# tum-pbs/PhiFlow

Hardware: NVIDIA H100
Metric: smoke_plume_512^3_steps_per_sec (higher is better)
Workload: dtype f32

## Files before the change

### phiflow_b200/csrc/ring_kernels.cu

```cuda
#include <cooperative_groups.h>
#include <type_traits>
#include "cg_common.cuh"
#include <cstdlib>
#include <cstring>
#include "launch.cuh"

namespace cg = cooperative_groups;

#define RING_CONSUMERS 256
#define RING_THREADS (RING_CONSUMERS + 32)
#define RING_MAX_STAGES 8
#define RING_G 4

struct RingCfg {
    int TY, R, pitch, nx4;
    int stage_floats;
    int ZC, nyt, nzc;
    int units_per_batch, total_units;
    int consumers;
    int groups;
    int shfl_ok;
    int hint;
    int merge;
    int dbg;
// ... 677 lines not shown
    {
        const float4 m = make_float4(c.x + q.x, c.y + q.y, c.z + q.z, c.w + q.w);
        e(off, c, m, nvalid, e0, e1, e2);
    }
};

template <int DIM, bool AXPY, bool GENERIC>
__global__ void __launch_bounds__(RING_THREADS, 2)
k_laplace_ring(DGrid g, DField f, RingCfg cfg, const float* __restrict__ x, float* __restrict__ y, float coeff)
{
    extern __shared__ __align__(128) unsigned char smem[];
    Ring rg;
    ring_init(rg, smem, cfg);
    ThreadGroups tg;
    groups_init(tg, cfg, g, f);
    const float* hsrc[2] = {x, nullptr};
    const float* esrc[2] = {nullptr, nullptr};
    REpiLaplace<AXPY> epi{y, coeff};
    for (int unit = blockIdx.x; unit < cfg.total_units; unit += gridDim.x) {
        const RingUnit u = ring_unit<DIM>(cfg, g, unit);
        ring_process_unit<GENERIC, DIM, 1, 0, false>(rg, cfg, g, f, tg, hsrc, esrc, 0.f, u, epi);
    }
}

struct CgRingArgs {
    CgArgs a;
    RingCfg cfg;
    int ring_smem_offset;
    int comm_merge;
    CommDev cm;
    float* d2;
    CgOperator op;
};

template <int DIM, bool GENERIC, CgOp OP, int NH, int NE, class Epi>
__device__ __forceinline__ void cg_op_unit(Ring& rg, const CgRingArgs& A, ThreadGroups& tg, const float* const* hsrc,
                                           const float* const* esrc, float beta, const RingUnit& u, Epi& epi)
{
    if constexpr (OP == CgOp::Helmholtz) {
        REpiHelm<Epi> he{epi, A.op.amount};
        ring_process_unit<GENERIC, DIM, NH, NE, true, OP>(rg, A.cfg, A.a.g, A.a.pf, tg, hsrc, esrc, beta, u, he);
    } else if constexpr (OP == CgOp::HelmholtzVarying) {
        REpiVarHelm<Epi> he{epi};
        ring_process_unit<GENERIC, DIM, NH, NE, true, OP>(rg, A.cfg, A.a.g, A.a.pf, tg, hsrc, esrc, beta, u, he, A.op.kbcast ? 0 : u.b, &A.op);
    } else ring_process_unit<GENERIC, DIM, NH, NE, true, OP>(rg, A.cfg, A.a.g, A.a.pf, tg, hsrc, esrc, beta, u, epi);
}

__device__ __forceinline__ unsigned long long ld_acquire_sys(const unsigned long long* p)
{
    unsigned long long v;
    asm volatile("ld.acquire.sys.global.u64 %0, [%1];" : "=l"(v) : "l"(p) : "memory");
    return v;
}
__device__ __forceinline__ void st_release_sys(unsigned long long* p, unsigned long long v)
{
    asm volatile("st.release.sys.global.u64 [%0], %1;" ::"l"(p), "l"(v) : "memory");
}

__device__ __forceinline__ bool comm_allreduce(const CommDev& cm, const CgShared& sh, int batch, unsigned long long seq)
{
    const int par = (int)(seq & 1ull);
    const size_t stride = 2 * (size_t)CG_MAX_BATCH;
    if (blockIdx.x == 0) {
        for (int q = 0; q < cm.n; ++q) {
            double* dst = cm.mbox[q] + ((size_t)par * PHI_MAX_RANKS + cm.rank) * stride;
            for (int b = threadIdx.x; b < batch; b += blockDim.x) { dst[b] = sh.sum0[b]; dst[CG_MAX_BATCH + b] = sh.sum1[b]; }
        }
        __threadfence_system();
        __syncthreads();
        if ((int)threadIdx.x < cm.n) st_release_sys(cm.flag[threadIdx.x] + par * PHI_MAX_RANKS + cm.rank, seq);
    }
    bool ok = true;
    if ((int)threadIdx.x < cm.n) {
        const unsigned long long* f = cm.flag[cm.rank] + par * PHI_MAX_RANKS + threadIdx.x;
        const long long t0 = clock64();
        while (ld_acquire_sys(f) < seq) {
            if (clock64() - t0 > 40000000000ll) { ok = false; break; }
        }
    }
    ok = __syncthreads_and(ok);
    const double* src = cm.mbox[cm.rank] + (size_t)par * PHI_MAX_RANKS * stride;
    for (int b = threadIdx.x; b < batch; b += blockDim.x) {
        double s0 = 0, s1 = 0;
        for (int q = 0; q < cm.n; ++q) {
            s0 += *(volatile const double*)(src + q * stride + b);
            s1 += *(volatile const double*)(src + q * stride + CG_MAX_BATCH + b);
        }
        sh.sum0[b] = s0; sh.sum1[b] = s1;
    }
    __syncthreads();
    return ok;
}

__device__ __forceinline__ bool comm_barrier_allreduce(const CommDev& cm, const CgShared& sh, const double* partials, int region, int batch,
                                                       int units_per_batch, const unsigned char* active, unsigned long long seq)
{
    const int par = (int)(seq & 1ull);
    const size_t stride = 2 * (size_t)CG_MAX_BATCH;
    __threadfence_system();
    __syncthreads();
    if (threadIdx.x == 0) {
        const unsigned prev = atomicAdd(cm.arrive, 1u);
        sh.any_cont[1] = ((prev + 1u) % gridDim.x == 0u) ? 1 : 0;
    }
    __syncthreads();
    if (sh.any_cont[1]) {
        __threadfence();
        reduce_partials(sh, partials, region, batch, units_per_batch, active);
        for (int q = 0; q < cm.n; ++q) {
            double* dst = cm.mbox[q] + ((size_t)par * PHI_MAX_RANKS + cm.rank) * stride;
            for (int b = threadIdx.x; b < batch; b += blockDim.x) { dst[b] = sh.sum0[b]; dst[CG_MAX_BATCH + b] = sh.sum1[b]; }
        }
        __threadfence_system();
        __syncthreads();
        if ((int)threadIdx.x < cm.n) st_release_sys(cm.flag[threadIdx.x] + par * PHI_MAX_RANKS + cm.rank, seq);
    }
    bool ok = true;
    if ((int)threadIdx.x < cm.n) {
        const unsigned long long* f = cm.flag[cm.rank] + par * PHI_MAX_RANKS + threadIdx.x;
        const long long t0 = clock64();
        while (ld_acquire_sys(f) < seq) {
            if (clock64() - t0 > 40000000000ll) { ok = false; break; }
        }
    }
    ok = __syncthreads_and(ok);
    const double* src = cm.mbox[cm.rank] + (size_t)par * PHI_MAX_RANKS * stride;
    for (int b = threadIdx.x; b < batch; b += blockDim.x) {
        double s0 = 0, s1 = 0;
        for (int q = 0; q < cm.n; ++q) {
            s0 += *(volatile const double*)(src + q * stride + b);
            s1 += *(volatile const double*)(src + q * stride + CG_MAX_BATCH + b);
        }
        sh.sum0[b] = s0; sh.sum1[b] = s1;
    }
    __syncthreads();
    return ok;
}

template <int DIM, class F>
__device__ __forceinline__ void ring_unit_cells(const RingCfg& cfg, const DGrid& g, const DField& pf, const ThreadGroups& tg,
                                                const RingUnit& u, F&& fn)
{
    if ((int)threadIdx.x >= cfg.consumers) return;
    long long plane_off = (long long)u.b * pf.sb + (long long)u.y0 * pf.sy + (DIM == 3 ? (long long)u.z0 * pf.sz : 0);
    for (int z = u.z0; z < u.z1; ++z, plane_off += pf.sz)
#pragma unroll
        for (int k = 0; k < RING_G; ++k) {
            if (tg.j[k] < 0 || u.y0 + tg.j[k] >= g.n[1]) continue;
            const int x0 = tg.eoff[k] - tg.j[k] * cfg.pitch;
            fn(plane_off + tg.goff[k], min(4, g.n[0] - x0));
        }
}

#define RING_GF 3
#define FUSED_TILE_BUFS 3

struct FusedGroups {
    int t[RING_GF];
    int tl[RING_GF], tr[RING_GF];
    int goff[RING_GF];
    unsigned valid, inner, needl, needr;
};

__device__ __forceinline__ void fused_groups_init(FusedGroups& fg, const RingCfg& cfg, const DGrid& g, const DField& pf)
{
    const int lane = threadIdx.x & 31, nx = g.n[0], pitch = cfg.pitch;
    fg.valid = fg.inner = fg.needl = fg.needr = 0;
#pragma unroll
    for (int k = 0; k < RING_GF; ++k) {
        const int ge = threadIdx.x + k * cfg.consumers;
        const int jj = ge / cfg.nx4, x0 = (ge - jj * cfg.nx4) * 4;
        const int row = jj * pitch;
        if (jj < cfg.TY + 2) fg.valid |= 1u << k;
        if (jj >= 1 && jj <= cfg.TY) fg.inner |= 1u << k;
        fg.t[k] = row + x0;
        fg.goff[k] = (jj - 1) * (int)pf.sy + x0;
        fg.tl[k] = row + x0 - 1; fg.tr[k] = row + x0 + 4;
        if (lane == 0) fg.needl |= 1u << k;
        if (lane == 31) fg.needr |= 1u << k;
        if (x0 == 0) { fg.needl |= 1u << k; fg.tl[k] = pf.klo[0] == PHI_BC_PERIODIC ? row + nx - 1 : row; }
        if (x0 + 4 >= nx) { fg.needr |= 1u << k; fg.tr[k] = pf.khi[0] == PHI_BC_PERIODIC ? row : row + nx - 1; }
        if (!(fg.needl & (1u << k))) fg.tl[k] = 0;
        if (!(fg.needr & (1u << k))) fg.tr[k] = 0;
    }
}

struct ProdUnitF {
    long long yoff[4];
    const float* base[4];
    uint32_t dsto[4];
    uint32_t nbytes[4];
    unsigned m[3];
    int tot[3];
};

__device__ __forceinline__ void prod_fused_setup(ProdUnitF& pu, const RingCfg& cfg, const DGrid& g, const DField& pf,
                                                 const float* d, const float* dprev, const float* x, int b, int y0)
{
    const int lane = threadIdx.x & 31, TY = cfg.TY;
    const uint32_t row_bytes = (uint32_t)cfg.pitch * 4u;
    const bool mergeable = cfg.merge && pf.sy == cfg.pitch;
    const int rows[3] = {TY + 4, TY + 2, TY};
    const int ylo[3] = {y0 - 2, y0 - 1, y0};
    const float* src[3] = {d, dprev, x};
    int cnt[3] = {0, 0, 0};
    pu.m[0] = pu.m[1] = pu.m[2] = 0;
#pragma unroll
    for (int it = 0; it < 4; ++it) {
        const int line = lane + 32 * it;
        pu.yoff[it] = 0; pu.base[it] = nullptr; pu.dsto[it] = 0; pu.nbytes[it] = row_bytes;
        int key = -1, yv = 0, first = 0;
#pragma unroll
        for (int arr = 0; arr < 3; ++arr) {
            if (key < 0 && line >= first && line < first + rows[arr] && src[arr]) {
                int yy = ylo[arr] + (line - first); float cv;
                phi_resolve(yy, pf, 1, cv);
                pu.yoff[it] = (long long)b * pf.sb + (long long)yy * pf.sy;
                pu.base[it] = src[arr];
                pu.dsto[it] = 4u * (uint32_t)(line * cfg.pitch);
                key = arr; yv = yy;
            }
            first += rows[arr];
        }
        cnt[0] += key == 0; cnt[1] += key == 1; cnt[2] += key == 2;
        const int pkey = __shfl_up_sync(0xffffffffu, key, 1), pyv = __shfl_up_sync(0xffffffffu, yv, 1);
        const bool cont = mergeable && key >= 0 && lane > 0 && pkey == key && pyv + 1 == yv;
        const unsigned cm = __ballot_sync(0xffffffffu, cont);
        if (key >= 0 && !cont) {
            const unsigned follow = lane == 31 ? 0u : (cm >> (lane + 1));
            pu.nbytes[it] = (uint32_t)__ffs(~follow) * row_bytes;
            if (key == 0) pu.m[0] |= 1u << it; else if (key == 1) pu.m[1] |= 1u << it; else pu.m[2] |= 1u << it;
        }
    }
#pragma unroll
    for (int c = 0; c < 3; ++c) {
#pragma unroll
        for (int o = 16; o > 0; o >>= 1) cnt[c] += __shfl_xor_sync(0xffffffffu, cnt[c], o);
        pu.tot[c] = cnt[c];
    }
}

__device__ __forceinline__ void ring_produce_fused(Ring& rg, const RingCfg& cfg, const DField& pf, const ProdUnitF& pu, int z, bool pplane, bool eplane)
{
    const int lane = threadIdx.x & 31;
    const int slot = rg.pos.slot;
    const uint32_t full = rg.full0 + 8 * slot;
    const uint32_t sbase = rg.stage0_s + 4u * (uint32_t)(slot * cfg.stage_floats);
    float cv;
    phi_resolve(z, pf, 2, cv);
    const long long zoff = (long long)z * pf.sz;
    const unsigned mask = pu.m[0] | (pplane ? pu.m[1] : 0u) | (eplane ? pu.m[2] : 0u);
    const int cnt = pu.tot[0] + (pplane ? pu.tot[1] : 0) + (eplane ? pu.tot[2] : 0);
    if (lane == 0) {
        mbar_wait(rg.empty0 + 8 * slot, rg.pos.par ^ 1u);
        mbar_expect_tx(full, (uint32_t)cnt * (uint32_t)cfg.pitch * 4u);
    }
    __syncwarp();
#pragma unroll
    for (int it = 0; it < 4; ++it)
        if (mask & (1u << it)) bulk_g2s(sbase + pu.dsto[it], pu.base[it] + pu.yoff[it] + zoff, pu.nbytes[it], full);
    rg.pos.next(cfg.R);
}

__device__ __forceinline__ float4 lds4(const float* s, int off) { return *reinterpret_cast<const float4*>(s + off); }
__device__ __forceinline__ float dot4(const float4& a, const float4& b) { return a.x * b.x + a.y * b.y + a.z * b.z + a.w * b.w; }

__device__ __forceinline__ float4 stencil7(const float4& c, float xl, float xr, const float4& ym, const float4& yp, const float4& zm, const float4& zp,
                                           float ix2, float iy2, float iz2, float cc)
{
    float4 q;
    q.x = fmaf(ix2, xl + c.y, fmaf(iy2, ym.x + yp.x, -cc * c.x));
    q.y = fmaf(ix2, c.x + c.z, fmaf(iy2, ym.y + yp.y, -cc * c.y));
    q.z = fmaf(ix2, c.y + c.w, fmaf(iy2, ym.z + yp.z, -cc * c.z));
    q.w = fmaf(ix2, c.z + xr, fmaf(iy2, ym.w + yp.w, -cc * c.w));
    q.x = fmaf(iz2, zm.x + zp.x, q.x);
    q.y = fmaf(iz2, zm.y + zp.y, q.y);
    q.z = fmaf(iz2, zm.z + zp.z, q.z);
    q.w = fmaf(iz2, zm.w + zp.w, q.w);
    return q;
}

struct FusedPass {
    const float* d; const float* dprev;
    float* dn; float* x;
    float alpha, aprev, beta, bprev;
};

__device__ __forceinline__ void ring_fused_unit(Ring& rg, const RingCfg& cfg, const DGrid& g, const DField& pf, const FusedGroups& fg,
                                                const FusedPass& P, float* tile, const RingUnit& u, float (&acc)[4])
{
    const int nz = u.z1 - u.z0;
    if ((int)threadIdx.x >= cfg.consumers) {
        ProdUnitF pu;
        prod_fused_setup(pu, cfg, g, pf, P.d, P.dprev, P.x, u.b, u.y0);
        for (int p = 0; p < nz + 4; ++p)
            ring_produce_fused(rg, cfg, pf, pu, u.z0 - 2 + p, p >= 1 && p <= nz + 2, P.x && p >= 2 && p <= nz + 1);
        return;
    }
    const int pitch = cfg.pitch, TY = cfg.TY;
    const int pb = (TY + 4) * pitch, xb = (2 * TY + 6) * pitch - pitch;
    const int tsz = (TY + 2) * pitch;
    const float ix2 = g.inv_dx2[0], iy2 = g.inv_dx2[1], iz2 = g.inv_dx2[2];
    const float cc = 2.f * (ix2 + iy2 + iz2);
    const float alpha = P.alpha, aprev = P.aprev, beta = P.beta, bprev = P.bprev;
    const bool has_prev = P.dprev != nullptr;
    long long plane_off = (long long)u.b * pf.sb + (long long)u.y0 * pf.sy + (long long)u.z0 * pf.sz - pf.sz;

    float4 dm[RING_GF], dc[RING_GF];
    float4 n2[RING_GF], n1[RING_GF];
    float4 r1[RING_GF];
    SlotIt cur = rg.pos, nxt = cur; nxt.next(cfg.R);
    ring_wait_full(rg, cur); ring_wait_full(rg, nxt);
    {
        const float* s0 = ring_ptr(rg, cfg, cur);
        const float* s1 = ring_ptr(rg, cfg, nxt);
#pragma unroll
        for (int k = 0; k < RING_GF; ++k) {
            dm[k] = f4_splat(0.f); dc[k] = f4_splat(0.f);
            if (fg.valid & (1u << k)) { dm[k] = lds4(s0, pitch + fg.t[k]); dc[k] = lds4(s1, pitch + fg.t[k]); }
            n2[k] = n1[k] = r1[k] = f4_splat(0.f);
        }
    }
    ring_release(rg, cur);
    cur = nxt; nxt.next(cfg.R);
    for (int i = 0; i < nz + 2; ++i) {
        const bool own = i >= 1 && i <= nz;
        ring_wait_full(rg, nxt);
        const float* sc = ring_ptr(rg, cfg, cur);
        const float* sn = ring_ptr(rg, cfg, nxt);
        float* tw = tile + (i % FUSED_TILE_BUFS) * tsz;
        float4 n0[RING_GF], r0[RING_GF];
#pragma unroll
        for (int k = 0; k < RING_GF; ++k) {
            n0[k] = r0[k] = f4_splat(0.f);
            if (!(fg.valid & (1u << k))) continue;
            const int o = pitch + fg.t[k];
            const float4 c = dc[k];
            const float4 ym = lds4(sc, o - pitch), yp = lds4(sc, o + pitch), zp = lds4(sn, o);
            float xl = __shfl_up_sync(0xffffffffu, c.w, 1), xr = __shfl_down_sync(0xffffffffu, c.x, 1);
            const float el = sc[pitch + fg.tl[k]], er = sc[pitch + fg.tr[k]];
            xl = (fg.needl & (1u << k)) ? el : xl;
            xr = (fg.needr & (1u << k)) ? er : xr;
            const float4 q = stencil7(c, xl, xr, ym, yp, dm[k], zp, ix2, iy2, iz2, cc);
            float4 rv = c, dp = f4_splat(0.f);
            if (has_prev) {
                dp = lds4(sc, pb + fg.t[k]);
                rv = make_float4(fmaf(-bprev, dp.x, c.x), fmaf(-bprev, dp.y, c.y), fmaf(-bprev, dp.z, c.z), fmaf(-bprev, dp.w, c.w));
            }
            rv.x = fmaf(-alpha, q.x, rv.x); rv.y = fmaf(-alpha, q.y, rv.y); rv.z = fmaf(-alpha, q.z, rv.z); rv.w = fmaf(-alpha, q.w, rv.w);
            const float4 dv = make_float4(fmaf(beta, c.x, rv.x), fmaf(beta, c.y, rv.y), fmaf(beta, c.z, rv.z), fmaf(beta, c.w, rv.w));
            *reinterpret_cast<float4*>(tw + fg.t[k]) = dv;
            if (own && (fg.inner & (1u << k))) {
                const long long off = plane_off + fg.goff[k];
                *reinterpret_cast<float4*>(P.dn + off) = dv;
                acc[1] += dot4(rv, rv);
                if (P.x) {
                    float4 xv = lds4(sc, xb + fg.t[k]);
                    xv.x += aprev * dp.x; xv.y += aprev * dp.y; xv.z += aprev * dp.z; xv.w += aprev * dp.w;
                    xv.x += alpha * c.x; xv.y += alpha * c.y; xv.z += alpha * c.z; xv.w += alpha * c.w;
                    *reinterpret_cast<float4*>(P.x + off) = xv;
                }
            }
            n0[k] = dv; r0[k] = rv;
            dm[k] = c; dc[k] = zp;
        }
        ring_release(rg, cur);
        asm volatile("bar.sync 1, %0;" ::"r"(cfg.consumers) : "memory");
        if (i >= 2) {
            const float* tp = tile + ((i - 1) % FUSED_TILE_BUFS) * tsz;
#pragma unroll
            for (int k = 0; k < RING_GF; ++k) {
                if (!(fg.inner & (1u << k))) continue;
                const float4 c = n1[k];
                const float4 ym = lds4(tp, fg.t[k] - pitch), yp = lds4(tp, fg.t[k] + pitch);
                float xl = __shfl_up_sync(0xffffffffu, c.w, 1), xr = __shfl_down_sync(0xffffffffu, c.x, 1);
                const float el = tp[fg.tl[k]], er = tp[fg.tr[k]];
                xl = (fg.needl & (1u << k)) ? el : xl;
                xr = (fg.needr & (1u << k)) ? er : xr;
                const float4 q = stencil7(c, xl, xr, ym, yp, n2[k], n0[k], ix2, iy2, iz2, cc);
                acc[0] += dot4(c, q);
                acc[2] += dot4(r1[k], q);
                acc[3] += dot4(q, q);
            }
        }
#pragma unroll
        for (int k = 0; k < RING_GF; ++k) { n2[k] = n1[k]; n1[k] = n0[k]; r1[k] = r0[k]; }
        cur = nxt; nxt.next(cfg.R);
        plane_off += pf.sz;
    }
    ring_release(rg, cur);
    rg.pos = nxt;
    asm volatile("bar.sync 1, %0;" ::"r"(cfg.consumers) : "memory");
}

struct REpiFusedStart {
    float* d; float acc0, acc1;
    __device__ __forceinline__ void set_plane(int, int) {}
    __device__ __forceinline__ void set_acc(const float4&) {}
    __device__ __forceinline__ void operator()(long long off, const float4& c, const float4& q, int, const float4&, const float4&, const float4&)
    {
        *reinterpret_cast<float4*>(d + off) = c;
        acc0 += dot4(c, q);
        acc1 += dot4(q, q);
    }
};

template <int DIM, bool GENERIC, bool DIST, bool ADAPT, CgOp OP = CgOp::Poisson, bool FUSED = false>
__global__ void __launch_bounds__(RING_THREADS, 1)
k_cg_ring(CgRingArgs A)
{
    constexpr bool MASK = OP == CgOp::Masked;
    static_assert((OP != CgOp::Helmholtz && OP != CgOp::HelmholtzVarying) || (!DIST && !ADAPT && !FUSED),
                  "the Helmholtz operators run on the single-GPU two-sweep CG only");
    static_assert(!MASK || !ADAPT || (!DIST && !FUSED), "CG-adaptive with obstacles runs on the single-GPU two-sweep CG only");
    static_assert(!cg_op_xslot(OP) || GENERIC, "the face-minimum stencil runs on the generic consumer");
    extern __shared__ __align__(128) unsigned char smem_raw[];
    const CgArgs& a = A.a;
    const RingCfg& cfg = A.cfg;
    CgShared sh = cg_carve(smem_raw, a.g.batch);
    Ring rg;
    ring_init(rg, smem_raw + A.ring_smem_offset, cfg);
    cg::grid_group grid = cg::this_grid();
    const DGrid& g = a.g;
    const int batch = g.batch;
    const double cells = (double)g.n[0] * g.n[1] * g.n[2] * (A.cm.n > 1 ? A.cm.n : 1);
    const float coffs = a.prm.matrix_offset;
    constexpr bool adaptive = ADAPT;
    int region = 0;
    ThreadGroups tg;
    groups_init(tg, cfg, g, a.pf);

    auto sweep = [&](const unsigned char* active, auto&& body) {
        int cur_b = cfg.split ? 0 : -1; float acc0 = 0.f, acc1 = 0.f;
        RingUnit u;
        for (int k = 0; ring_next_unit<DIM>(cfg, g, k, u); ++k) {
            if (active && !active[u.b]) continue;
            if (u.b != cur_b) {
                if (cur_b >= 0) flush_partials(sh, a.partials, region, batch, cur_b, acc0, acc1);
                cur_b = u.b; acc0 = 0.f; acc1 = 0.f;
            }
            body(u, acc0, acc1);
        }
        if (cur_b >= 0) flush_partials(sh, a.partials, region, batch, cur_b, acc0, acc1);
    };
    const CommDev& cm = A.cm;
    unsigned long long seq = cm.n > 1 ? *cm.seq : 0ull;
    bool comm_ok = true;
    auto barrier_and_reduce = [&](const unsigned char* active) {
        fence_proxy_async();
        if (DIST && cm.n > 1 && A.comm_merge) {
            comm_ok = comm_barrier_allreduce(cm, sh, a.partials, region, batch, cfg.split ? (int)gridDim.x : cfg.units_per_batch, active, ++seq) && comm_ok;
            region ^= 1;
            fence_proxy_async();
            return;
        }
        if (cm.n > 1) __threadfence_system();
        grid.sync();
        fence_proxy_async();
        reduce_partials(sh, a.partials, region, batch, cfg.split ? (int)gridDim.x : cfg.units_per_batch, active);
        region ^= 1;
        if (cm.n > 1) {
            comm_ok = comm_allreduce(cm, sh, batch, ++seq) && comm_ok;
            fence_proxy_async();
        }
    };
    const long long nzsz = (long long)g.n[2] * a.pf.sz;
    using PH = typename std::conditional<DIST, PeerHalo, NoPeerHalo>::type;
    auto peer_halo = [&](float* lo_arr, float* hi_arr) {
        PH ph;
        if constexpr (DIST) {
            ph.plo = cm.lower >= 0 ? lo_arr + nzsz : nullptr;
            ph.phi = cm.upper >= 0 ? hi_arr - nzsz : nullptr;
        }
        ph.zf = 0;
        return ph;
    };

    for (int b = threadIdx.x; b < batch; b += blockDim.x) { sh.mean[b] = 0.f; sh.offs[b] = 0.f; }
    __syncthreads();

    if (a.prm.balance_rhs || coffs != 0.f) {
        sweep(nullptr, [&](const RingUnit& u, float& acc0, float& acc1) {
            ring_unit_cells<DIM>(cfg, g, a.pf, tg, u, [&](long long off, int nvalid) {
                for (int j = 0; j < nvalid; ++j) { acc0 += a.rhs[off + j]; acc1 += MASK ? a.acc[off + j] : a.x[off + j]; }
            });
        });
        barrier_and_reduce(nullptr);
        for (int b = threadIdx.x; b < batch; b += blockDim.x) {
            if (MASK) { sh.mean[b] = (a.prm.balance_rhs && sh.sum1[b] > 0.0) ? (float)(sh.sum0[b] / sh.sum1[b]) : 0.f; sh.offs[b] = 0.f; }
            else { sh.mean[b] = a.prm.balance_rhs ? (float)(sh.sum0[b] / cells) : 0.f; sh.offs[b] = coffs * (float)sh.sum1[b]; }
        }
        __syncthreads();
    }

    {
        const float* hsrc[2] = {a.x, (OP == CgOp::Masked ? a.acc : (OP == CgOp::HelmholtzVarying ? A.op.k : nullptr))};
        const float* esrc[2] = {a.rhs, nullptr};
        sweep(nullptr, [&](const RingUnit& u, float& acc0, float& acc1) {
            REpiResidual0<PH> epi{a.r, sh.mean[u.b], sh.offs[u.b], 0.f, 0.f, peer_halo(cm.lo_r, cm.hi_r), adaptive};
            if constexpr (OP == CgOp::Poisson) ring_process_unit<GENERIC, DIM, 1, 1>(rg, cfg, g, a.pf, tg, hsrc, esrc, 0.f, u, epi);
            else cg_op_unit<DIM, GENERIC, OP, 1, 1>(rg, A, tg, hsrc, esrc, 0.f, u, epi);
            acc0 += epi.acc0; acc1 += epi.acc1;
        });
    }
    barrier_and_reduce(nullptr);
    for (int b = threadIdx.x; b < batch; b += blockDim.x) {
        const double d0 = sh.sum0[b], d0tol = sh.sum1[b];
        sh.delta[b] = d0;
        const float tol = fmaxf(a.prm.rtol * a.prm.rtol * (float)d0tol, a.prm.atol * a.prm.atol);
        sh.tol_sq[b] = tol; sh.rsq0[b] = (float)d0;
        const bool conv = (float)d0 <= tol;
        const bool divg = !isfinite((float)d0);
        sh.conv[b] = conv; sh.divg[b] = divg; sh.iters[b] = 0;
        sh.cont[b] = (!conv && !divg && a.prm.max_iter > 0) ? 1 : 0;
        sh.beta[b] = 0.f; sh.alpha[b] = 0.f; sh.aprev[b] = 0.f;
    }
    __syncthreads();
    if (threadIdx.x == 0) { int any = 0; for (int b = 0; b < batch; ++b) any |= sh.cont[b]; *sh.any_cont = any; }
    __syncthreads();

    if constexpr (FUSED) {
        static_assert(DIM == 3 && !GENERIC && !DIST && !ADAPT && OP == CgOp::Poisson, "the one-sweep CG is 3-D, branch-free, single-GPU CG only");
        float* const D[3] = {a.d0, a.d1, A.d2};
        float* const tile = rg.stage0 + (size_t)cfg.R * cfg.stage_floats;
        FusedGroups fg;
        fused_groups_init(fg, cfg, g, a.pf);
        if (*sh.any_cont) {
            const float* hsrc[2] = {a.r, nullptr};
            const float* esrc[2] = {nullptr, nullptr};
            sweep(sh.cont, [&](const RingUnit& u, float& acc0, float& acc1) {
                REpiFusedStart epi{D[0], 0.f, 0.f};
                ring_process_unit<false, 3, 1, 0, true>(rg, cfg, g, a.pf, tg, hsrc, esrc, 0.f, u, epi);
                acc0 += epi.acc0; acc1 += epi.acc1;
            });
            barrier_and_reduce(sh.cont);
            for (int b = threadIdx.x; b < batch; b += blockDim.x) {
                if (!sh.cont[b]) continue;
                const double dl = sh.delta[b], dq = sh.sum0[b];
                const float al = (dq != 0.0) ? (float)(dl / dq) : 0.f;
// ... 207 lines not shown
static const int kSmemBudget = 227 * 1024;
#define RING_UNIT_OVERHEAD 2.5

static bool ring_config(const DGrid& g, int lines_a, int lines_b, int reserve_bytes, int min_stages, int max_stages,
                        int target_units, RingCfg* out, int consumers = RING_CONSUMERS, int zhalo = 2)
{
    RingCfg c;
    c.split = 0; c.Zm = 0; c.split_t = 0;
    c.consumers = consumers;
    c.pitch = g.cext[0]; c.nx4 = g.cext[0] / 4;
    const int row_bytes = c.pitch * 4;
    int ty = g.dim == 3 ? 4 : 16;
    if (g.dim == 3) {
        const int want = 2048 / (g.cext[0] > 0 ? g.cext[0] : 1);
        ty = 1;
        while (ty * 2 <= want && ty < 16) ty *= 2;
        while (ty > 1 && ty / 2 >= g.n[1]) ty /= 2;
    }
    if (const char* e = getenv("PHICUDA_RING_TY")) { const int v = atoi(e); if (v >= 1 && v <= 32) ty = v; }
    for (;; ty /= 2) {
        if (ty < 1) return false;
        if (ty * c.nx4 > RING_G * consumers) continue;
        if (lines_a * ty + lines_b > 128) continue;
        const int stage_bytes = (lines_a * ty + lines_b) * row_bytes;
        const int r = (kSmemBudget - reserve_bytes - 128) / stage_bytes;
        if (const char* e = getenv("PHICUDA_RING_R")) { const int v = atoi(e); if (v >= min_stages && v < max_stages) max_stages = v; }
        if (r >= min_stages) { c.TY = ty; c.R = r > max_stages ? max_stages : r; c.stage_floats = stage_bytes / 4; break; }
    }
    while (g.dim == 2 && c.TY > 1 && c.TY / 2 >= g.n[1]) c.TY /= 2;
    c.groups = (c.TY * c.nx4 + consumers - 1) / consumers;
    c.shfl_ok = (c.nx4 % 32 == 0) ? 1 : 0;
    { const char* e = getenv("PHICUDA_RING_HINT"); c.hint = (e && e[0] == '1') ? 1 : 0; }
    { const char* e = getenv("PHICUDA_RING_MERGE"); c.merge = (e && e[0] == '0') ? 0 : 1; }
    { const char* e = getenv("PHICUDA_RING_DEBUG"); c.dbg = e ? atoi(e) : 0; }
    if (g.dim == 3) {
        c.nyt = (g.n[1] + c.TY - 1) / c.TY;
        const int ctas = target_units;
        double best = -1.0; int best_nzc = 1;
        const int max_nzc = g.n[2] >= 4 ? g.n[2] / 4 : 1;
        for (int nzc = 1; nzc <= max_nzc; ++nzc) {
            const int zc = (g.n[2] + nzc - 1) / nzc;
            if ((g.n[2] + zc - 1) / zc != nzc) continue;
            const long long units = (long long)c.nyt * nzc * g.batch;
            const long long rounds = (units + ctas - 1) / ctas;
            const double util = (double)units / (double)(rounds * ctas);
            const double score = util / (1.0 + (zhalo + RING_UNIT_OVERHEAD) / zc);
            if (score > best + 1e-9) { best = score; best_nzc = nzc; }
        }
        if (const char* e = getenv("PHICUDA_RING_NZC")) {
            const int v = atoi(e);
            if (v >= 1 && v <= g.n[2]) { const int zc = (g.n[2] + v - 1) / v; best_nzc = (g.n[2] + zc - 1) / zc; }
        }
        c.nzc = best_nzc; c.ZC = (g.n[2] + best_nzc - 1) / best_nzc;
        c.units_per_batch = c.nyt * c.nzc;
        c.total_units = c.units_per_batch * g.batch;
    } else {
        c.nyt = (g.n[1] + c.TY - 1) / c.TY; c.nzc = 1; c.ZC = 1;
        c.units_per_batch = c.nyt; c.total_units = c.nyt * g.batch;
    }
    *out = c;
    return true;
}

static bool ring_all_fast(const DGrid& g, const DField& f, const RingCfg& c)
{
    if (!c.shfl_ok || c.nx4 * 4 != g.n[0] || c.TY * c.nx4 != c.groups * c.consumers || g.n[1] % c.TY != 0) return false;
    for (int a = 0; a < g.dim; ++a) if (f.klo[a] == PHI_BC_CONST || f.khi[a] == PHI_BC_CONST) return false;
    return c.groups == 1 || c.groups == 2 || c.groups == 4;
}

static void note_ring_launch(int kernel, const RingCfg& c, bool generic, bool dist, bool adaptive, int grid, bool masked = false)
{
    PhiLaunchInfo li; memset(&li, 0, sizeof(li));
    li.kernel = kernel; li.generic = generic; li.dist = dist; li.adaptive = adaptive; li.masked = masked;
    li.TY = c.TY; li.stages = c.R; li.ZC = c.ZC; li.nzc = c.nzc; li.groups = c.groups; li.total_units = c.total_units; li.grid_ctas = grid; li.split = c.split;
    phi_note_launch(li);
}

int phi_launch_laplace_ring(const DGrid& g, const DField& f, const float* x, float* y, float coeff, bool axpy, cudaStream_t s)
{
    RingCfg cfg;
    const int sms = phi_sm_count();
    if (!ring_config(g, 1, 2, kSmemBudget / 2 + 1024, g.dim == 3 ? 4 : 2, 6, sms * 2, &cfg)) return -100;
    const size_t smem = 128 + (size_t)cfg.R * cfg.stage_floats * 4;
    int grid = sms * 2;
    if (grid > cfg.total_units) grid = cfg.total_units;
    cudaError_t e;
    const bool generic = !ring_all_fast(g, f, cfg);
#define LAUNCH_LAP(D, AX, GEN) do { \
        e = cudaFuncSetAttribute(k_laplace_ring<D, AX, GEN>, cudaFuncAttributeMaxDynamicSharedMemorySize, (int)smem); \
        if (e == cudaSuccess) k_laplace_ring<D, AX, GEN><<<grid, RING_THREADS, smem, s>>>(g, f, cfg, x, y, coeff); } while (0)
#define LAUNCH_LAP2(D, AX) do { if (generic) LAUNCH_LAP(D, AX, true); else LAUNCH_LAP(D, AX, false); } while (0)
    if (g.dim == 3) { if (axpy) LAUNCH_LAP2(3, true); else LAUNCH_LAP2(3, false); }
    else            { if (axpy) LAUNCH_LAP2(2, true); else LAUNCH_LAP2(2, false); }
#undef LAUNCH_LAP2
#undef LAUNCH_LAP
    if (e != cudaSuccess) return (int)e;
    note_ring_launch(PHI_KERNEL_LAPLACE_RING, cfg, generic, false, false, grid);
    return (int)cudaGetLastError();
}

static bool cg_ring_config(const DGrid& g, CgOp op, int cgs, int target_units, RingCfg* c)
{
    const bool xslot = cg_op_xslot(op);
    return ring_config(g, xslot ? 5 : 4, xslot ? 6 : 2, cgs, g.dim == 3 ? (xslot ? 3 : 4) : 2, RING_MAX_STAGES, target_units, c);
}

using CgRingKernel = void (*)(CgRingArgs);
static CgRingKernel cg_ring_kernel(CgOp op, int dim, bool generic, bool dist, bool adapt, bool fused)
{
    constexpr CgOp P = CgOp::Poisson, M = CgOp::Masked, H = CgOp::Helmholtz, V = CgOp::HelmholtzVarying;
    const bool d3 = dim == 3;
    switch (op) {
    case P:
        if (fused)
            return d3 && !generic && !dist && !adapt ? k_cg_ring<3, false, false, false, P, true> : nullptr;
        if (d3) return generic ? (dist ? (adapt ? k_cg_ring<3, true, true, true> : k_cg_ring<3, true, true, false>)
                                       : (adapt ? k_cg_ring<3, true, false, true> : k_cg_ring<3, true, false, false>))
                               : (dist ? (adapt ? k_cg_ring<3, false, true, true> : k_cg_ring<3, false, true, false>)
                                       : (adapt ? k_cg_ring<3, false, false, true> : k_cg_ring<3, false, false, false>));
        return generic ? (dist ? (adapt ? k_cg_ring<2, true, true, true> : k_cg_ring<2, true, true, false>)
                               : (adapt ? k_cg_ring<2, true, false, true> : k_cg_ring<2, true, false, false>))
                       : (dist ? (adapt ? k_cg_ring<2, false, true, true> : k_cg_ring<2, false, true, false>)
                               : (adapt ? k_cg_ring<2, false, false, true> : k_cg_ring<2, false, false, false>));
    case M:
        if (!generic || fused || (adapt && dist)) return nullptr;
        if (adapt) return d3 ? k_cg_ring<3, true, false, true, M> : k_cg_ring<2, true, false, true, M>;
        return d3 ? (dist ? k_cg_ring<3, true, true, false, M> : k_cg_ring<3, true, false, false, M>)
                  : (dist ? k_cg_ring<2, true, true, false, M> : k_cg_ring<2, true, false, false, M>);
    case H:
        if (dist || adapt || fused) return nullptr;
        return d3 ? (generic ? k_cg_ring<3, true, false, false, H> : k_cg_ring<3, false, false, false, H>)
                  : (generic ? k_cg_ring<2, true, false, false, H> : k_cg_ring<2, false, false, false, H>);
    case V:
        if (dist || adapt || fused || !generic) return nullptr;
        return d3 ? k_cg_ring<3, true, false, false, V> : k_cg_ring<2, true, false, false, V>;
    }
    return nullptr;
}

int phi_launch_cg_ring(const CgLaunch& l, const CommDev* cm, cudaStream_t s)
{
    const DGrid& g = l.g;
    const CgOp op = l.op.kind;
    if (g.batch > CG_MAX_BATCH) return -100;
    if (op == CgOp::Masked && l.prm.matrix_offset != 0.f) return -100;
    const bool xslot = cg_op_xslot(op);
    CgRingArgs A;
    const int cgs = (int)((cg_smem_bytes(g.batch) + 127) / 128 * 128);
    const int sms = phi_sm_count();
    if (!cg_ring_config(g, op, cgs, sms, &A.cfg)) return -100;
    if (l.prm.method == PHI_SOLVER_CG_ADAPTIVE && !xslot && A.cfg.TY == 1
        && !ring_config(g, 4, 3, cgs, g.dim == 3 ? 4 : 2, RING_MAX_STAGES, sms, &A.cfg)) return -100;
    const int threads = RING_THREADS;
    A.ring_smem_offset = cgs;
    int per_sm = 0;
    cudaError_t e;
    const bool generic = xslot || !ring_all_fast(g, l.pf, A.cfg);
    const bool dist = cm && cm->n > 1;
    const bool adapt = l.prm.method == PHI_SOLVER_CG_ADAPTIVE;
    bool fused = false;
    size_t tile_bytes = 0;
    {
        const char* e = getenv("PHICUDA_CG_PASSES");
        const DField& pf = l.pf;
        if (!(e && atoi(e) == 2) && g.dim == 3 && !generic && !dist && !adapt && op == CgOp::Poisson && l.prm.matrix_offset == 0.f
            && pf.klo[1] == PHI_BC_PERIODIC && pf.khi[1] == PHI_BC_PERIODIC && pf.klo[2] == PHI_BC_PERIODIC && pf.khi[2] == PHI_BC_PERIODIC) {
            RingCfg fc;
            if (ring_config(g, 3, 6, cgs, 4, RING_MAX_STAGES, sms, &fc, RING_CONSUMERS, 4)
                && ring_config(g, 3, 6, cgs + FUSED_TILE_BUFS * (fc.TY + 2) * fc.pitch * 4, 4, RING_MAX_STAGES, sms, &fc, RING_CONSUMERS, 4)
                && ring_all_fast(g, pf, fc) && (fc.TY + 2) * fc.nx4 <= RING_GF * fc.consumers) {
                fused = true;
                A.cfg = fc;
                tile_bytes = (size_t)FUSED_TILE_BUFS * (fc.TY + 2) * fc.pitch * 4;
            }
        }
    }
    const size_t smem = (size_t)cgs + 128 + (size_t)A.cfg.R * A.cfg.stage_floats * 4 + tile_bytes;
    const void* fn = (const void*)cg_ring_kernel(op, g.dim, generic, dist, adapt, fused);
    if (!fn) return -100;
    e = cudaFuncSetAttribute(fn, cudaFuncAttributeMaxDynamicSharedMemorySize, (int)smem);
    if (e == cudaSuccess) e = cudaOccupancyMaxActiveBlocksPerMultiprocessor(&per_sm, fn, threads, smem);
    if (e != cudaSuccess || per_sm < 1) return -100;
    int grid = sms * per_sm;
    A.cfg.split = 0; A.cfg.Zm = 0; A.cfg.split_t = 0;
    {
        const char* e = getenv("PHICUDA_RING_SPLIT");
        const int force = e ? atoi(e) : -1;
        const int nyt = A.cfg.nyt, nz = g.n[2];
        const int zh = fused ? 4 : 2;
        if (g.dim == 3 && g.batch == 1 && force != 0 && grid <= CG_MAX_GRID && nyt < grid && nz >= 8) {
            const int spare = grid - nyt, T = (nyt + spare - 1) / spare;
            int best_zm = 0; double best = 1e30;
            for (int zm = 4; zm <= nz - 1; ++zm) {
                const double main_c = zm + zh + RING_UNIT_OVERHEAD, tail_c = T * (nz - zm + zh + RING_UNIT_OVERHEAD);
                const double cost = main_c > tail_c ? main_c : tail_c;
                if (cost < best) { best = cost; best_zm = zm; }
            }
            const long long rounds = ((long long)A.cfg.total_units + grid - 1) / grid;
            const double dflt = rounds * (A.cfg.ZC + zh + RING_UNIT_OVERHEAD);
            if (best_zm > 0 && (force == 1 || best < dflt * 0.97)) {
                A.cfg.split = 1; A.cfg.Zm = best_zm; A.cfg.split_t = T;
                A.cfg.nzc = 2; A.cfg.ZC = best_zm; A.cfg.units_per_batch = A.cfg.total_units = 2 * nyt;
            }
        }
    }
    if (!A.cfg.split && grid > A.cfg.total_units) grid = A.cfg.total_units;
    if (grid > CG_MAX_GRID) grid = CG_MAX_GRID;
    const CgWorkspace w = phi_cg_workspace(g, l.workspace);
    CgArgs& a = A.a;
    a.g = g; a.pf = l.pf; a.um = UnitMap();
    a.rhs = l.rhs; a.x = l.x; a.acc = l.op.mask;
    a.r = w.r; a.d0 = w.d0; a.d1 = w.d1; a.partials = w.partials;
    A.d2 = w.d2;
    A.op = l.op;
    a.result = l.result; a.prm = l.prm;
    if (cm) A.cm = *cm; else { memset(&A.cm, 0, sizeof(A.cm)); A.cm.n = 1; A.cm.lower = A.cm.upper = -1; }
    { const char* e = getenv("PHICUDA_COMM_MERGE"); A.comm_merge = (e && e[0] == '1') ? 1 : 0; }
    void* args[] = {&A};
    e = cudaLaunchCooperativeKernel(fn, dim3(grid), dim3(threads), args, smem, s);
    if (e != cudaSuccess) { phi_set_error("cg ring: cooperative launch failed: %s", cudaGetErrorString(e)); return (int)e; }
    note_ring_launch(PHI_KERNEL_CG_RING, A.cfg, generic, dist, adapt, grid, op == CgOp::Masked);
    phi_note_cg_passes(fused ? 1 : 2);
    phi_note_cg_operator(op == CgOp::HelmholtzVarying ? PHI_CG_OP_HELMHOLTZ_VARYING : (op == CgOp::Helmholtz ? PHI_CG_OP_HELMHOLTZ : PHI_CG_OP_POISSON));
    return 0;
}

struct HelmConsts { float clo[3][3], chi[3][3]; };

__global__ void k_helm_bias(DGrid g, DField f, int C, float amount, HelmConsts hc, const float* __restrict__ y, float* __restrict__ out)
{
    const long long plane = (long long)g.n[0] * g.n[1], cells = plane * g.n[2], total = cells * g.batch;
    for (long long i = blockIdx.x * (long long)blockDim.x + threadIdx.x; i < total; i += (long long)gridDim.x * blockDim.x) {
        const int b = (int)(i / cells);
        const long long r = i - b * cells;
        const int z = (int)(r / plane), yy = (int)((r - z * plane) / g.n[0]), x = (int)(r - z * plane - (long long)yy * g.n[0]);
        const int idx[3] = {x, yy, z};
        const int c = b % C;
        float lap = 0.f;
        for (int ax = 0; ax < g.dim; ++ax) {
            float gs = 0.f;
            if (idx[ax] == 0 && f.klo[ax] == PHI_BC_CONST) gs += hc.clo[c][ax];
            if (idx[ax] == g.n[ax] - 1 && f.khi[ax] == PHI_BC_CONST) gs += hc.chi[c][ax];
            lap += gs * g.inv_dx2[ax];
        }
        const long long off = b * f.sb + z * f.sz + (long long)yy * f.sy + x;
        out[off] = fmaf(amount, lap, y[off]);
    }
}

__global__ void k_helm_bias_var(DGrid g, DField f, float ndt, HelmConsts hc, const float* __restrict__ k, int kbcast,
                                const float* __restrict__ y, float* __restrict__ out)
{
    const long long plane = (long long)g.n[0] * g.n[1], cells = plane * g.n[2], total = cells * g.batch;
    for (long long i = blockIdx.x * (long long)blockDim.x + threadIdx.x; i < total; i += (long long)gridDim.x * blockDim.x) {
        const int b = (int)(i / cells);
        const long long r = i - b * cells;
        const int z = (int)(r / plane), yy = (int)((r - z * plane) / g.n[0]), x = (int)(r - z * plane - (long long)yy * g.n[0]);
        const int idx[3] = {x, yy, z};
        const long long cell = z * f.sz + (long long)yy * f.sy + x;
        const float w = __fmul_rn(ndt, k[(kbcast ? 0 : b) * f.sb + cell]);
        float bias = 0.f;
        for (int ax = 0; ax < g.dim; ++ax) {
            float s = 0.f;
            if (idx[ax] == 0 && f.klo[ax] == PHI_BC_CONST) { const float c = hc.clo[0][ax]; s += fminf(w, c) * c; }
            if (idx[ax] == g.n[ax] - 1 && f.khi[ax] == PHI_BC_CONST) { const float c = hc.chi[0][ax]; s += fminf(w, c) * c; }
            bias += s * g.inv_dx2[ax];
        }
        const long long off = b * f.sb + cell;
        out[off] = y[off] - bias;
    }
}

bool phi_cg_ring_fits(const DGrid& g, CgOp op)
{
    if (g.batch > CG_MAX_BATCH || g.halo != 0) return false;
    RingCfg c;
    return cg_ring_config(g, op, (int)((cg_smem_bytes(g.batch) + 127) / 128 * 128), 1, &c);
}

int phi_cg_ring_max_width(const DGrid& g, CgOp op, bool adapt)
{
    if (g.batch > CG_MAX_BATCH || g.halo != 0) return 0;
    const int cgs = (int)((cg_smem_bytes(g.batch) + 127) / 128 * 128);
    for (int w = g.cext[0] < 4096 ? g.cext[0] / 4 * 4 : 4096; w >= 4; w -= 4) {
        DGrid h = g; h.n[0] = w; h.cext[0] = w;
        RingCfg c;
        if (!cg_ring_config(h, op, cgs, 1, &c)) continue;
        if (adapt && !cg_op_xslot(op) && c.TY == 1 && !ring_config(h, 4, 3, cgs, h.dim == 3 ? 4 : 2, RING_MAX_STAGES, 1, &c)) continue;
        return w;
    }
    return 0;
}

int phi_launch_diffuse_implicit(const CgLaunch& l, int C, const DField* cf, cudaStream_t s)
{
    const DGrid& g = l.g;
    const bool varying = l.op.kind == CgOp::HelmholtzVarying;
    HelmConsts hc;
    bool bias = false;
    for (int c = 0; c < 3; ++c)
        for (int ax = 0; ax < 3; ++ax) {
            const bool used = c < C && ax < g.dim;
            hc.clo[c][ax] = used && cf[c].klo[ax] == PHI_BC_CONST ? cf[c].clo[ax] : 0.f;
            hc.chi[c][ax] = used && cf[c].khi[ax] == PHI_BC_CONST ? cf[c].chi[ax] : 0.f;
            bias = bias || hc.clo[c][ax] != 0.f || hc.chi[c][ax] != 0.f;
        }
    CgLaunch m = l;
    if (bias && (varying || l.op.amount != 0.f)) {
        float* yb = phi_cg_workspace(g, l.workspace).d2;
        const long long total = (long long)g.n[0] * g.n[1] * g.n[2] * g.batch;
        const long long want = (total + 255) / 256, cap = (long long)phi_sm_count() * 8;
        const int blocks = (int)(want < cap ? want : cap);
        if (varying) k_helm_bias_var<<<blocks, 256, 0, s>>>(g, l.pf, l.op.ndt, hc, l.op.k, l.op.kbcast, l.rhs, yb);
        else k_helm_bias<<<blocks, 256, 0, s>>>(g, l.pf, C, l.op.amount, hc, l.rhs, yb);
        const cudaError_t e = cudaGetLastError();
        if (e != cudaSuccess) return (int)e;
        m.rhs = yb;
    }
    return phi_launch_cg_ring(m, nullptr, s);
}
```

Measured before the change: 1.883.

## Split fused CG ring groups into inner/halo and stream x directly from global

Restructures the fused CG ring kernel's thread-to-cell mapping into separate inner-row groups and y-halo groups, so inner rows no longer need per-group inner masks and halo rows do only the direction update. The x vector is no longer staged through the TMA ring. Each consumer prefetches its own x values for the next plane from global with streaming loads, which shrinks ring stage traffic. Edge (x-boundary) handling is simplified to lane-based selection. The risk is extra register pressure from the prefetched x values and halo state, and x loads that are no longer asynchronous.

Measured after the change: 1.981 (median of 6 runs). +5.2%, better.

```diff
diff --git a/phiflow_b200/csrc/ring_kernels.cu b/phiflow_b200/csrc/ring_kernels.cu
--- a/phiflow_b200/csrc/ring_kernels.cu
+++ b/phiflow_b200/csrc/ring_kernels.cu
@@ -853,36 +853,44 @@
         }
 }
 
-#define RING_GF 3
+#define FUSED_GI 2
+#define FUSED_GH 2
 #define FUSED_TILE_BUFS 3
 
 struct FusedGroups {
-    int t[RING_GF];
-    int tl[RING_GF], tr[RING_GF];
-    int goff[RING_GF];
-    unsigned valid, inner, needl, needr;
+    int ti[FUSED_GI], th[FUSED_GH];
+    int ei[FUSED_GI], eh[FUSED_GH];
+    int gi[FUSED_GI];
+    unsigned vi, vh;
 };
 
 __device__ __forceinline__ void fused_groups_init(FusedGroups& fg, const RingCfg& cfg, const DGrid& g, const DField& pf)
 {
-    const int lane = threadIdx.x & 31, nx = g.n[0], pitch = cfg.pitch;
-    fg.valid = fg.inner = fg.needl = fg.needr = 0;
-#pragma unroll
-    for (int k = 0; k < RING_GF; ++k) {
+    const int lane = threadIdx.x & 31, nx = g.n[0], pitch = cfg.pitch, nx4 = cfg.nx4;
+    auto edge = [&](int jj, int x0) -> int {
+        const int row = jj * pitch;
+        if (lane == 0) return x0 == 0 ? (pf.klo[0] == PHI_BC_PERIODIC ? row + nx - 1 : row) : row + x0 - 1;
+        if (lane == 31) return x0 + 4 >= nx ? (pf.khi[0] == PHI_BC_PERIODIC ? row : row + nx - 1) : row + x0 + 4;
+        return 0;
+    };
+    fg.vi = fg.vh = 0;
+#pragma unroll
+    for (int k = 0; k < FUSED_GI; ++k) {
         const int ge = threadIdx.x + k * cfg.consumers;
-        const int jj = ge / cfg.nx4, x0 = (ge - jj * cfg.nx4) * 4;
-        const int row = jj * pitch;
-        if (jj < cfg.TY + 2) fg.valid |= 1u << k;
-        if (jj >= 1 && jj <= cfg.TY) fg.inner |= 1u << k;
-        fg.t[k] = row + x0;
-        fg.goff[k] = (jj - 1) * (int)pf.sy + x0;
-        fg.tl[k] = row + x0 - 1; fg.tr[k] = row + x0 + 4;
-        if (lane == 0) fg.needl |= 1u << k;
-        if (lane == 31) fg.needr |= 1u << k;
-        if (x0 == 0) { fg.needl |= 1u << k; fg.tl[k] = pf.klo[0] == PHI_BC_PERIODIC ? row + nx - 1 : row; }
-        if (x0 + 4 >= nx) { fg.needr |= 1u << k; fg.tr[k] = pf.khi[0] == PHI_BC_PERIODIC ? row : row + nx - 1; }
-        if (!(fg.needl & (1u << k))) fg.tl[k] = 0;
-        if (!(fg.needr & (1u << k))) fg.tr[k] = 0;
+        const int j = ge / nx4, x0 = (ge - j * nx4) * 4;
+        if (j < cfg.TY) fg.vi |= 1u << k;
+        fg.ti[k] = (j + 1) * pitch + x0;
+        fg.ei[k] = edge(j + 1, x0);
+        fg.gi[k] = j * (int)pf.sy + x0;
+    }
+#pragma unroll
+    for (int k = 0; k < FUSED_GH; ++k) {
+        const int ge = threadIdx.x + k * cfg.consumers;
+        const int h = ge / nx4, x0 = (ge - h * nx4) * 4;
+        const int jj = h == 0 ? 0 : cfg.TY + 1;
+        if (h < 2) fg.vh |= 1u << k;
+        fg.th[k] = jj * pitch + x0;
+        fg.eh[k] = edge(jj, x0);
     }
 }
 
@@ -891,28 +899,28 @@
     const float* base[4];
     uint32_t dsto[4];
     uint32_t nbytes[4];
-    unsigned m[3];
-    int tot[3];
+    unsigned m[2];
+    int tot[2];
 };
 
 __device__ __forceinline__ void prod_fused_setup(ProdUnitF& pu, const RingCfg& cfg, const DGrid& g, const DField& pf,
-                                                 const float* d, const float* dprev, const float* x, int b, int y0)
+                                                 const float* d, const float* dprev, int b, int y0)
 {
     const int lane = threadIdx.x & 31, TY = cfg.TY;
     const uint32_t row_bytes = (uint32_t)cfg.pitch * 4u;
     const bool mergeable = cfg.merge && pf.sy == cfg.pitch;
-    const int rows[3] = {TY + 4, TY + 2, TY};
-    const int ylo[3] = {y0 - 2, y0 - 1, y0};
-    const float* src[3] = {d, dprev, x};
-    int cnt[3] = {0, 0, 0};
-    pu.m[0] = pu.m[1] = pu.m[2] = 0;
+    const int rows[2] = {TY + 4, TY + 2};
+    const int ylo[2] = {y0 - 2, y0 - 1};
+    const float* src[2] = {d, dprev};
+    int cnt[2] = {0, 0};
+    pu.m[0] = pu.m[1] = 0;
 #pragma unroll
     for (int it = 0; it < 4; ++it) {
         const int line = lane + 32 * it;
         pu.yoff[it] = 0; pu.base[it] = nullptr; pu.dsto[it] = 0; pu.nbytes[it] = row_bytes;
         int key = -1, yv = 0, first = 0;
 #pragma unroll
-        for (int arr = 0; arr < 3; ++arr) {
+        for (int arr = 0; arr < 2; ++arr) {
             if (key < 0 && line >= first && line < first + rows[arr] && src[arr]) {
                 int yy = ylo[arr] + (line - first); float cv;
                 phi_resolve(yy, pf, 1, cv);
@@ -923,25 +931,25 @@
             }
             first += rows[arr];
         }
-        cnt[0] += key == 0; cnt[1] += key == 1; cnt[2] += key == 2;
+        cnt[0] += key == 0; cnt[1] += key == 1;
         const int pkey = __shfl_up_sync(0xffffffffu, key, 1), pyv = __shfl_up_sync(0xffffffffu, yv, 1);
         const bool cont = mergeable && key >= 0 && lane > 0 && pkey == key && pyv + 1 == yv;
         const unsigned cm = __ballot_sync(0xffffffffu, cont);
         if (key >= 0 && !cont) {
             const unsigned follow = lane == 31 ? 0u : (cm >> (lane + 1));
             pu.nbytes[it] = (uint32_t)__ffs(~follow) * row_bytes;
-            if (key == 0) pu.m[0] |= 1u << it; else if (key == 1) pu.m[1] |= 1u << it; else pu.m[2] |= 1u << it;
-        }
-    }
-#pragma unroll
-    for (int c = 0; c < 3; ++c) {
+            pu.m[key] |= 1u << it;
+        }
+    }
+#pragma unroll
+    for (int c = 0; c < 2; ++c) {
 #pragma unroll
         for (int o = 16; o > 0; o >>= 1) cnt[c] += __shfl_xor_sync(0xffffffffu, cnt[c], o);
         pu.tot[c] = cnt[c];
     }
 }
 
-__device__ __forceinline__ void ring_produce_fused(Ring& rg, const RingCfg& cfg, const DField& pf, const ProdUnitF& pu, int z, bool pplane, bool eplane)
+__device__ __forceinline__ void ring_produce_fused(Ring& rg, const RingCfg& cfg, const DField& pf, const ProdUnitF& pu, int z, bool pplane)
 {
     const int lane = threadIdx.x & 31;
     const int slot = rg.pos.slot;
@@ -950,8 +958,8 @@
     float cv;
     phi_resolve(z, pf, 2, cv);
     const long long zoff = (long long)z * pf.sz;
-    const unsigned mask = pu.m[0] | (pplane ? pu.m[1] : 0u) | (eplane ? pu.m[2] : 0u);
-    const int cnt = pu.tot[0] + (pplane ? pu.tot[1] : 0) + (eplane ? pu.tot[2] : 0);
+    const unsigned mask = pu.m[0] | (pplane ? pu.m[1] : 0u);
+    const int cnt = pu.tot[0] + (pplane ? pu.tot[1] : 0);
     if (lane == 0) {
         mbar_wait(rg.empty0 + 8 * slot, rg.pos.par ^ 1u);
         mbar_expect_tx(full, (uint32_t)cnt * (uint32_t)cfg.pitch * 4u);
@@ -993,33 +1001,57 @@
     const int nz = u.z1 - u.z0;
     if ((int)threadIdx.x >= cfg.consumers) {
         ProdUnitF pu;
-        prod_fused_setup(pu, cfg, g, pf, P.d, P.dprev, P.x, u.b, u.y0);
+        prod_fused_setup(pu, cfg, g, pf, P.d, P.dprev, u.b, u.y0);
         for (int p = 0; p < nz + 4; ++p)
-            ring_produce_fused(rg, cfg, pf, pu, u.z0 - 2 + p, p >= 1 && p <= nz + 2, P.x && p >= 2 && p <= nz + 1);
+            ring_produce_fused(rg, cfg, pf, pu, u.z0 - 2 + p, p >= 1 && p <= nz + 2);
         return;
     }
     const int pitch = cfg.pitch, TY = cfg.TY;
-    const int pb = (TY + 4) * pitch, xb = (2 * TY + 6) * pitch - pitch;
+    const int pb = (TY + 4) * pitch;
     const int tsz = (TY + 2) * pitch;
+    const int lane = threadIdx.x & 31;
     const float ix2 = g.inv_dx2[0], iy2 = g.inv_dx2[1], iz2 = g.inv_dx2[2];
     const float cc = 2.f * (ix2 + iy2 + iz2);
     const float alpha = P.alpha, aprev = P.aprev, beta = P.beta, bprev = P.bprev;
     const bool has_prev = P.dprev != nullptr;
     long long plane_off = (long long)u.b * pf.sb + (long long)u.y0 * pf.sy + (long long)u.z0 * pf.sz - pf.sz;
 
-    float4 dm[RING_GF], dc[RING_GF];
-    float4 n2[RING_GF], n1[RING_GF];
-    float4 r1[RING_GF];
+    auto dnew = [&](const float* sc, const float* sn, int o, int e, const float4& c, const float4& zm, float4& rv, float4& dp, float4& zp) {
+        const float4 ym = lds4(sc, o - pitch), yp = lds4(sc, o + pitch);
+        zp = lds4(sn, o);
+        float xl = __shfl_up_sync(0xffffffffu, c.w, 1), xr = __shfl_down_sync(0xffffffffu, c.x, 1);
+        const float ev = sc[pitch + e];
+        if (lane == 0) xl = ev;
+        if (lane == 31) xr = ev;
+        const float4 q = stencil7(c, xl, xr, ym, yp, zm, zp, ix2, iy2, iz2, cc);
+        rv = c; dp = f4_splat(0.f);
+        if (has_prev) {
+            dp = lds4(sc, pb + o - pitch);
+            rv = make_float4(fmaf(-bprev, dp.x, c.x), fmaf(-bprev, dp.y, c.y), fmaf(-bprev, dp.z, c.z), fmaf(-bprev, dp.w, c.w));
+        }
+        rv.x = fmaf(-alpha, q.x, rv.x); rv.y = fmaf(-alpha, q.y, rv.y); rv.z = fmaf(-alpha, q.z, rv.z); rv.w = fmaf(-alpha, q.w, rv.w);
+        return make_float4(fmaf(beta, c.x, rv.x), fmaf(beta, c.y, rv.y), fmaf(beta, c.z, rv.z), fmaf(beta, c.w, rv.w));
+    };
+
+    float4 dm[FUSED_GI], dc[FUSED_GI];
+    float4 hm[FUSED_GH], hc[FUSED_GH];
+    float4 n2[FUSED_GI], n1[FUSED_GI];
+    float4 r1[FUSED_GI];
+    float4 xv[FUSED_GI];
     SlotIt cur = rg.pos, nxt = cur; nxt.next(cfg.R);
     ring_wait_full(rg, cur); ring_wait_full(rg, nxt);
     {
         const float* s0 = ring_ptr(rg, cfg, cur);
         const float* s1 = ring_ptr(rg, cfg, nxt);
 #pragma unroll
-        for (int k = 0; k < RING_GF; ++k) {
-            dm[k] = f4_splat(0.f); dc[k] = f4_splat(0.f);
-            if (fg.valid & (1u << k)) { dm[k] = lds4(s0, pitch + fg.t[k]); dc[k] = lds4(s1, pitch + fg.t[k]); }
-            n2[k] = n1[k] = r1[k] = f4_splat(0.f);
+        for (int k = 0; k < FUSED_GI; ++k) {
+            dm[k] = dc[k] = n2[k] = n1[k] = r1[k] = xv[k] = f4_splat(0.f);
+            if (fg.vi & (1u << k)) { dm[k] = lds4(s0, pitch + fg.ti[k]); dc[k] = lds4(s1, pitch + fg.ti[k]); }
+        }
+#pragma unroll
+        for (int k = 0; k < FUSED_GH; ++k) {
+            hm[k] = hc[k] = f4_splat(0.f);
+            if (fg.vh & (1u << k)) { hm[k] = lds4(s0, pitch + fg.th[k]); hc[k] = lds4(s1, pitch + fg.th[k]); }
         }
     }
     ring_release(rg, cur);
@@ -1030,54 +1062,56 @@
         const float* sc = ring_ptr(rg, cfg, cur);
         const float* sn = ring_ptr(rg, cfg, nxt);
         float* tw = tile + (i % FUSED_TILE_BUFS) * tsz;
-        float4 n0[RING_GF], r0[RING_GF];
-#pragma unroll
-        for (int k = 0; k < RING_GF; ++k) {
+#pragma unroll
+        for (int k = 0; k < FUSED_GH; ++k) {
+            if (!(fg.vh & (1u << k))) continue;
+            float4 rv, dp, zp;
+            const float4 dv = dnew(sc, sn, pitch + fg.th[k], fg.eh[k], hc[k], hm[k], rv, dp, zp);
+            *reinterpret_cast<float4*>(tw + fg.th[k]) = dv;
+            hm[k] = hc[k]; hc[k] = zp;
+        }
+        float4 n0[FUSED_GI], r0[FUSED_GI];
+        float* const dnp = P.dn + plane_off;
+        float* const xp = P.x ? P.x + plane_off : nullptr;
+#pragma unroll
+        for (int k = 0; k < FUSED_GI; ++k) {
             n0[k] = r0[k] = f4_splat(0.f);
-            if (!(fg.valid & (1u << k))) continue;
-            const int o = pitch + fg.t[k];
+            if (!(fg.vi & (1u << k))) continue;
             const float4 c = dc[k];
-            const float4 ym = lds4(sc, o - pitch), yp = lds4(sc, o + pitch), zp = lds4(sn, o);
-            float xl = __shfl_up_sync(0xffffffffu, c.w, 1), xr = __shfl_down_sync(0xffffffffu, c.x, 1);
-            const float el = sc[pitch + fg.tl[k]], er = sc[pitch + fg.tr[k]];
-            xl = (fg.needl & (1u << k)) ? el : xl;
-            xr = (fg.needr & (1u << k)) ? er : xr;
-            const float4 q = stencil7(c, xl, xr, ym, yp, dm[k], zp, ix2, iy2, iz2, cc);
-            float4 rv = c, dp = f4_splat(0.f);
-            if (has_prev) {
-                dp = lds4(sc, pb + fg.t[k]);
-                rv = make_float4(fmaf(-bprev, dp.x, c.x), fmaf(-bprev, dp.y, c.y), fmaf(-bprev, dp.z, c.z), fmaf(-bprev, dp.w, c.w));
-            }
-            rv.x = fmaf(-alpha, q.x, rv.x); rv.y = fmaf(-alpha, q.y, rv.y); rv.z = fmaf(-alpha, q.z, rv.z); rv.w = fmaf(-alpha, q.w, rv.w);
-            const float4 dv = make_float4(fmaf(beta, c.x, rv.x), fmaf(beta, c.y, rv.y), fmaf(beta, c.z, rv.z), fmaf(beta, c.w, rv.w));
-            *reinterpret_cast<float4*>(tw + fg.t[k]) = dv;
-            if (own && (fg.inner & (1u << k))) {
-                const long long off = plane_off + fg.goff[k];
-                *reinterpret_cast<float4*>(P.dn + off) = dv;
+            float4 rv, dp, zp;
+            const float4 dv = dnew(sc, sn, pitch + fg.ti[k], fg.ei[k], c, dm[k], rv, dp, zp);
+            *reinterpret_cast<float4*>(tw + fg.ti[k]) = dv;
+            if (own) {
+                *reinterpret_cast<float4*>(dnp + fg.gi[k]) = dv;
                 acc[1] += dot4(rv, rv);
-                if (P.x) {
-                    float4 xv = lds4(sc, xb + fg.t[k]);
-                    xv.x += aprev * dp.x; xv.y += aprev * dp.y; xv.z += aprev * dp.z; xv.w += aprev * dp.w;
-                    xv.x += alpha * c.x; xv.y += alpha * c.y; xv.z += alpha * c.z; xv.w += alpha * c.w;
-                    *reinterpret_cast<float4*>(P.x + off) = xv;
+                if (xp) {
+                    float4 x4 = xv[k];
+                    x4.x += aprev * dp.x; x4.y += aprev * dp.y; x4.z += aprev * dp.z; x4.w += aprev * dp.w;
+                    x4.x += alpha * c.x; x4.y += alpha * c.y; x4.z += alpha * c.z; x4.w += alpha * c.w;
+                    *reinterpret_cast<float4*>(xp + fg.gi[k]) = x4;
                 }
             }
             n0[k] = dv; r0[k] = rv;
             dm[k] = c; dc[k] = zp;
         }
         ring_release(rg, cur);
+        if (xp && i < nz) {
+#pragma unroll
+            for (int k = 0; k < FUSED_GI; ++k)
+                if (fg.vi & (1u << k)) xv[k] = __ldcs(reinterpret_cast<const float4*>(xp + pf.sz + fg.gi[k]));
+        }
         asm volatile("bar.sync 1, %0;" ::"r"(cfg.consumers) : "memory");
         if (i >= 2) {
             const float* tp = tile + ((i - 1) % FUSED_TILE_BUFS) * tsz;
 #pragma unroll
-            for (int k = 0; k < RING_GF; ++k) {
-                if (!(fg.inner & (1u << k))) continue;
+            for (int k = 0; k < FUSED_GI; ++k) {
+                if (!(fg.vi & (1u << k))) continue;
                 const float4 c = n1[k];
-                const float4 ym = lds4(tp, fg.t[k] - pitch), yp = lds4(tp, fg.t[k] + pitch);
+                const float4 ym = lds4(tp, fg.ti[k] - pitch), yp = lds4(tp, fg.ti[k] + pitch);
                 float xl = __shfl_up_sync(0xffffffffu, c.w, 1), xr = __shfl_down_sync(0xffffffffu, c.x, 1);
-                const float el = tp[fg.tl[k]], er = tp[fg.tr[k]];
-                xl = (fg.needl & (1u << k)) ? el : xl;
-                xr = (fg.needr & (1u << k)) ? er : xr;
+                const float ev = tp[fg.ei[k]];
+                if (lane == 0) xl = ev;
+                if (lane == 31) xr = ev;
                 const float4 q = stencil7(c, xl, xr, ym, yp, n2[k], n0[k], ix2, iy2, iz2, cc);
                 acc[0] += dot4(c, q);
                 acc[2] += dot4(r1[k], q);
@@ -1085,7 +1119,7 @@
             }
         }
 #pragma unroll
-        for (int k = 0; k < RING_GF; ++k) { n2[k] = n1[k]; n1[k] = n0[k]; r1[k] = r0[k]; }
+        for (int k = 0; k < FUSED_GI; ++k) { n2[k] = n1[k]; n1[k] = n0[k]; r1[k] = r0[k]; }
         cur = nxt; nxt.next(cfg.R);
         plane_off += pf.sz;
     }
@@ -1599,7 +1633,6 @@
     if (!cg_ring_config(g, op, cgs, sms, &A.cfg)) return -100;
     if (l.prm.method == PHI_SOLVER_CG_ADAPTIVE && !xslot && A.cfg.TY == 1
         && !ring_config(g, 4, 3, cgs, g.dim == 3 ? 4 : 2, RING_MAX_STAGES, sms, &A.cfg)) return -100;
-    const int threads = RING_THREADS;
     A.ring_smem_offset = cgs;
     int per_sm = 0;
     cudaError_t e;
@@ -1616,13 +1649,14 @@
             RingCfg fc;
             if (ring_config(g, 3, 6, cgs, 4, RING_MAX_STAGES, sms, &fc, RING_CONSUMERS, 4)
                 && ring_config(g, 3, 6, cgs + FUSED_TILE_BUFS * (fc.TY + 2) * fc.pitch * 4, 4, RING_MAX_STAGES, sms, &fc, RING_CONSUMERS, 4)
-                && ring_all_fast(g, pf, fc) && (fc.TY + 2) * fc.nx4 <= RING_GF * fc.consumers) {
+                && ring_all_fast(g, pf, fc) && fc.TY * fc.nx4 <= FUSED_GI * fc.consumers && 2 * fc.nx4 <= FUSED_GH * fc.consumers) {
                 fused = true;
                 A.cfg = fc;
                 tile_bytes = (size_t)FUSED_TILE_BUFS * (fc.TY + 2) * fc.pitch * 4;
             }
         }
     }
+    const int threads = RING_THREADS;
     const size_t smem = (size_t)cgs + 128 + (size_t)A.cfg.R * A.cfg.stage_floats * 4 + tile_bytes;
     const void* fn = (const void*)cg_ring_kernel(op, g.dim, generic, dist, adapt, fused);
     if (!fn) return -100;
```
